# juliohm/GeoStatsSolvers.jl

Hardware: AMD Instinct MI355X
Metric: kriged domain points/sec (OK, 1000 3-D data, Matern-3/2, global neighbourhood) (higher is better)
Workload: dtype f64; 1 GPU; configs[1]: OK, 1000 3-D data -> 1000000 domain points per GPU, Matern-3/2 range 30, global neighbourhood; step = device fit + predict; points_per_gpu=1000000, ndata=1000, factor=replicated

## Files before the change

### geostatssolvers.jl_amd/csrc/krig.hip

```cpp
#include "gss_internal.h"
#include "cokrig.h"

#include <mutex>
#include "mfma_f64.h"

#include <cmath>
#include <cstdlib>
#include <cstring>
#include <type_traits>
#include <vector>

namespace gss {

constexpr int MAX_NC = 64;
constexpr int NSEG = 4;

struct DriftSpec {
  int variant;
  int nc;
  int dim;
  signed char e[MAX_NC][3];
  double center[3];
  double inv_scale[3];
};

template <int DIM>
__global__ __launch_bounds__(256) void drift_rows_kernel(DriftSpec ds, const double* __restrict__ x,
                                                         const double* __restrict__ drift_vals, int64_t npts,
                                                         int64_t ncols_pad, double* __restrict__ out, int64_t ld,
                                                         int nrows) {
  const int64_t p = (int64_t)blockIdx.x * 256 + threadIdx.x;
  if (p >= ncols_pad) return;
  const int64_t pc = p < npts ? p : npts - 1;
  double xs[DIM];
#pragma unroll
  for (int k = 0; k < DIM; ++k) xs[k] = (x[pc * DIM + k] - ds.center[k]) * ds.inv_scale[k];
  for (int c = 0; c < nrows; ++c) {
    double f = 0.0;
    if (c < ds.nc) {
      if (ds.variant == GSS_KRIG_ORDINARY) {
        f = 1.0;
      } else if (ds.variant == GSS_KRIG_UNIVERSAL) {
        f = 1.0;
#pragma unroll
        for (int k = 0; k < DIM; ++k)
          for (int q = 0; q < ds.e[c][k]; ++q) f *= xs[k];
      } else {
        f = drift_vals[pc * ds.nc + c];
      }
    }
    out[(int64_t)c * ld + p] = f;
  }
}

template <int KIND>
__device__ __forceinline__ double cov_d2_select(const VgDev& vg, double d2) {
  const double val = vg.cs * vg_shape(KIND, fmax(d2, 1e-300), vg.inv_range, vg.mscale, vg.pw);
  return d2 <= 0.0 ? vg.sill : val;
}

template <int DIM, int KIND>
__global__ __launch_bounds__(256) void krig_rhs2_kernel(VgDev vg, const double* __restrict__ xd, int n,
                                                        const double* __restrict__ x0, int64_t m_valid,
                                                        double* __restrict__ R, int64_t ldr, int seg_len, int nblk,
                                                        int64_t ncols) {
  for (int unit = blockIdx.x; unit < nblk * NSEG; unit += gridDim.x) {
    const int seg = unit % NSEG;
    const int64_t p = (int64_t)(unit / NSEG) * 512 + 2 * threadIdx.x;
    if (p >= ncols) continue;
    const int64_t pa = p < m_valid ? p : m_valid - 1, pb = p + 1 < m_valid ? p + 1 : m_valid - 1;
    double ca[DIM], cb[DIM];
#pragma unroll
    for (int k = 0; k < DIM; ++k) {
      ca[k] = x0[pa * DIM + k];
      cb[k] = x0[pb * DIM + k];
    }
    const int j0 = seg * seg_len;
    const int j1 = j0 + seg_len < n ? j0 + seg_len : n;
    double2* rp = reinterpret_cast<double2*>(R + (int64_t)j0 * ldr + p);
    const int64_t ld2 = ldr >> 1;
#pragma unroll 4
    for (int j = j0; j < j1; ++j) {
      double x[DIM];
#pragma unroll
      for (int k = 0; k < DIM; ++k) x[k] = xd[j * DIM + k];
      double2 v;
      if (KIND < 0) {
        v.x = cov_pair<DIM>(vg, x, ca);
        v.y = cov_pair<DIM>(vg, x, cb);
      } else {
        const double da = sqdist_nofma<DIM>(x, ca, vg.ir, true);
        const double db = sqdist_nofma<DIM>(x, cb, vg.ir, true);
        v.x = cov_d2_select < KIND < 0 ? 0 : KIND > (vg, da);
        v.y = cov_d2_select < KIND < 0 ? 0 : KIND > (vg, db);
      }
      *rp = v;
      rp += ld2;
    }
  }
}

template <int DIM>
static int32_t launch_krig_rhs(hipStream_t s, const VgDev& vg, const double* xd, int n, const double* x0,
                               int64_t m_valid, double* R, int64_t ldr, int seg_len, int nblk) {
  GSS_REQUIRE((ldr & 1) == 0, "launch_krig_rhs: odd leading dimension %lld (16-B stores need an even one)",
              (long long)ldr);
  const int64_t ncols = (int64_t)nblk * 256;
  const int nblk2 = (int)((ncols + 511) / 512);
  const dim3 g2((unsigned)(nblk2 * NSEG));
#define GSS_K1W_LAUNCH(KIND)                                                                                         \
  hipLaunchKernelGGL((krig_rhs2_kernel<DIM, KIND>), g2, dim3(256), 0, s, vg, xd, n, x0, m_valid, R, ldr, seg_len,    \
                     nblk2, ncols)
  switch (vg.nextra == 0 ? vg.kind : -1) {
    case GSS_VG_GAUSSIAN: GSS_K1W_LAUNCH(GSS_VG_GAUSSIAN); break;
    case GSS_VG_EXPONENTIAL: GSS_K1W_LAUNCH(GSS_VG_EXPONENTIAL); break;
    case GSS_VG_SPHERICAL: GSS_K1W_LAUNCH(GSS_VG_SPHERICAL); break;
    case VG_MATERN12: GSS_K1W_LAUNCH(VG_MATERN12); break;
    case VG_MATERN32: GSS_K1W_LAUNCH(VG_MATERN32); break;
    case VG_MATERN52: GSS_K1W_LAUNCH(VG_MATERN52); break;
    default: GSS_K1W_LAUNCH(-1); break;
  }
#undef GSS_K1W_LAUNCH
  return GSS_OK;
}


template <int DIM>
__global__ __launch_bounds__(256) void cokrig_system_kernel(VgDev vg, const double* __restrict__ xd,
                                                            const int* __restrict__ var,
                                                            const double* __restrict__ tab, int n,
                                                            double* __restrict__ M, int64_t ldw) {
  const int j = blockIdx.x * 256 + threadIdx.x;
  const int i0 = blockIdx.y * 64;
  const int i1 = i0 + 64 < n ? i0 + 64 : n;
  if (j >= n) return;
  double c[DIM];
#pragma unroll
  for (int k = 0; k < DIM; ++k) c[k] = xd[(int64_t)j * DIM + k];
  const int vj = var[j];
  for (int i = i0; i < i1; ++i) {
    double x[DIM];
#pragma unroll
    for (int k = 0; k < DIM; ++k) x[k] = xd[(int64_t)i * DIM + k];
    bool zero;
    const double rho = co_rho<DIM, -1>(vg, x, c, &zero);
    const int e = var[i] * CO_MAXZ + vj;
    M[(int64_t)i * ldw + j] = zero ? tab[CO_C0 + e] : tab[e] * rho;
  }
}

__global__ __launch_bounds__(256) void cokrig_indicator_kernel(const int* __restrict__ var, int n, int nc,
                                                               double* __restrict__ Fd) {
  const int i = blockIdx.x * 256 + threadIdx.x;
  if (i >= n) return;
  const int v = var[i];
  for (int c = 0; c < nc; ++c) Fd[(int64_t)c * n + i] = v == c ? 1.0 : 0.0;
}

__global__ __launch_bounds__(256) void cokrig_center_kernel(double* __restrict__ z, const int* __restrict__ var,
                                                            const double* __restrict__ tab, int n) {
  const int i = blockIdx.x * 256 + threadIdx.x;
  if (i < n) z[i] -= tab[CO_MEANS + var[i]];
}

template <int DIM, int KIND>
__global__ __launch_bounds__(256) void cokrig_rhs_kernel(VgDev vg, const double* __restrict__ xd,
                                                         const int* __restrict__ var, const double* __restrict__ tab,
// ... 185 lines not shown
  double macc[2] = {0.0, 0.0};

  int buf = 0;
  for (int I = Ibeg; I < Iend; ++I) {
    const int i0 = I * BM;
    const int tm_max = (N1 + 1 - i0 + 15) / 16 < 8 ? (N1 + 1 - i0 + 15) / 16 : 8;
    const int t0 = i0 / BK;

    const double* wp = W + (int64_t)kq * ldw + i0 + i2;
    const double* rp = R + (int64_t)kq * ldr + p0 + i2;
    if (I == Ibeg) {
      d2v ra[4], rb[4];
#pragma unroll
      for (int r = 0; r < 4; ++r) {
        ra[r] = *reinterpret_cast<const d2v*>(wp + (int64_t)(4 * r) * ldw);
        rb[r] = *reinterpret_cast<const d2v*>(rp + (int64_t)(4 * r) * ldr);
      }
#pragma unroll
      for (int r = 0; r < 4; ++r) {
        *reinterpret_cast<d2v*>(As + (kq + 4 * r) * LDS_LD + i2) = ra[r];
        *reinterpret_cast<d2v*>(Bs + (kq + 4 * r) * LDS_LD + i2) = rb[r];
      }
      __syncthreads();
    }

    auto row_block = [&](auto tmx) __attribute__((always_inline)) {
      constexpr int TM_MAX = decltype(tmx)::value;
      d4 accw[8][2];
#pragma unroll
      for (int tm = 0; tm < TM_MAX; ++tm) accw[tm][0] = accw[tm][1] = d4{0.0, 0.0, 0.0, 0.0};

      auto stage = [&](int t, auto tmn, auto is_last) __attribute__((always_inline)) {
        constexpr int TM_MIN = decltype(tmn)::value;
        constexpr bool last = decltype(is_last)::value;
        const int cur = buf;
        const bool more = !last || (I + 1 < Iend);
        d2v ra[4], rb[4];
        if (more) {
          const double* wq = last ? wp + BM : wp + (int64_t)(t + 1) * BK * ldw;
          const double* rq = last ? rp : rp + (int64_t)(t + 1) * BK * ldr;
#pragma unroll
          for (int r = 0; r < 4; ++r) {
            ra[r] = *reinterpret_cast<const d2v*>(wq + (int64_t)(4 * r) * ldw);
            rb[r] = *reinterpret_cast<const d2v*>(rq + (int64_t)(4 * r) * ldr);
          }
        }
        mma_stage_w14<TM_MIN, TM_MAX>(As + cur * TILE_LDS, Bs + cur * TILE_LDS, accw, wave, lane);
        if (more) {
          double* an = As + (cur ^ 1) * TILE_LDS;
          double* bn = Bs + (cur ^ 1) * TILE_LDS;
#pragma unroll
          for (int r = 0; r < 4; ++r) {
            *reinterpret_cast<d2v*>(an + (kq + 4 * r) * LDS_LD + i2) = ra[r];
            *reinterpret_cast<d2v*>(bn + (kq + 4 * r) * LDS_LD + i2) = rb[r];
          }
        }
        __syncthreads();
        buf ^= 1;
      };
      for (int t = 0; t < t0; ++t) stage(t, std::integral_constant<int, 0>{}, std::false_type{});
#define GSS_K3_DIAG_STAGE(S) \
  if constexpr (S < TM_MAX) stage(t0 + S, std::integral_constant<int, S>{}, std::bool_constant<S + 1 == TM_MAX>{})
      GSS_K3_DIAG_STAGE(0);
      GSS_K3_DIAG_STAGE(1);
      GSS_K3_DIAG_STAGE(2);
      GSS_K3_DIAG_STAGE(3);
      GSS_K3_DIAG_STAGE(4);
      GSS_K3_DIAG_STAGE(5);
      GSS_K3_DIAG_STAGE(6);
      GSS_K3_DIAG_STAGE(7);
#undef GSS_K3_DIAG_STAGE

#pragma unroll
      for (int tn = 0; tn < 2; ++tn) {
        double s = 0.0;
#pragma unroll
        for (int tm = 0; tm < TM_MAX; ++tm)
#pragma unroll
          for (int r = 0; r < 4; ++r) {
            const int row = i0 + tm * 16 + lk + 4 * r;
            const double v = accw[tm][tn][r];
            const double vv = v * v;
            s += (row < n) ? vv : (row < N1 ? -vv : 0.0);
            if (row == N1) macc[tn] += v;
          }
        qacc[tn] += s;
      }
    };
    switch (tm_max) {
      case 1: row_block(std::integral_constant<int, 1>{}); break;
      case 2: row_block(std::integral_constant<int, 2>{}); break;
      case 3: row_block(std::integral_constant<int, 3>{}); break;
      case 4: row_block(std::integral_constant<int, 4>{}); break;
      case 5: row_block(std::integral_constant<int, 5>{}); break;
      case 6: row_block(std::integral_constant<int, 6>{}); break;
      case 7: row_block(std::integral_constant<int, 7>{}); break;
      default: row_block(std::integral_constant<int, 8>{}); break;
    }
  }

#pragma unroll
  for (int tn = 0; tn < 2; ++tn) {
    qacc[tn] += __shfl_xor(qacc[tn], 16);
    qacc[tn] += __shfl_xor(qacc[tn], 32);
    macc[tn] += __shfl_xor(macc[tn], 16);
    macc[tn] += __shfl_xor(macc[tn], 32);
  }
  __syncthreads();
  double* red = smem;
  double* redm = smem + 2 * BN;
  if (lk == 0) {
    red[wave * 32 + lr] = qacc[0];
    red[wave * 32 + 16 + lr] = qacc[1];
    red[BN + wave * 32 + lr] = 0.0;
    red[BN + wave * 32 + 16 + lr] = 0.0;
    redm[wave * 32 + lr] = macc[0];
    redm[wave * 32 + 16 + lr] = macc[1];
    redm[BN + wave * 32 + lr] = 0.0;
    redm[BN + wave * 32 + 16 + lr] = 0.0;
  }
  __syncthreads();
  if (SPLIT) {
    if (tid < BN) {
      qpart[(int64_t)Ibeg * ldr + p0 + tid] = red[tid] + red[BN + tid];
      if (Ibeg == N1 / BM && p0 + tid < m_valid) mean_out[p0 + tid] = mean0 + (redm[tid] + redm[BN + tid]);
    }
    return;
  }
  if (tid < BN) {
    const int64_t p = p0 + tid;
    if (p < m_valid) {
      const double q = red[tid] + red[BN + tid];
      const double mu = mean0 + (redm[tid] + redm[BN + tid]);
      const double v = sill - q;
      mean_out[p] = mu;
      var_out[p] = v > 0.0 ? v : 0.0;
      if (status_out) status_out[p] = GSS_PT_OK;
    }
  }
}

__global__ __launch_bounds__(256) void krig_finish_kernel(const double* __restrict__ qpart, int nI, int64_t ldr,
                                                          double sill, int64_t m_valid, double* __restrict__ var_out,
                                                          uint8_t* __restrict__ status_out) {
  const int64_t p = (int64_t)blockIdx.x * 256 + threadIdx.x;
  if (p >= m_valid) return;
  double q = 0.0;
  for (int I = 0; I < nI; ++I) q += qpart[(int64_t)I * ldr + p];
  const double v = sill - q;
  var_out[p] = v > 0.0 ? v : 0.0;
  if (status_out) status_out[p] = GSS_PT_OK;
}

__global__ void flip_tail_kernel(double* u, int64_t from, int64_t to) {
  const int64_t i = from + (int64_t)blockIdx.x * 256 + threadIdx.x;
  if (i < to) u[i] = -u[i];
}

__global__ void flip_rows_kernel(double* u, int64_t ld, int64_t from, int64_t to, int64_t ncols) {
  const int64_t i = from + (int64_t)blockIdx.x * 256 + threadIdx.x;
  const int64_t c = blockIdx.y;
  if (i < to && c < ncols) u[i + c * ld] = -u[i + c * ld];
}

__global__ void add_scalar_kernel(double* x, int64_t n, double v) {
  const int64_t i = (int64_t)blockIdx.x * 256 + threadIdx.x;
  if (i < n) x[i] += v;
}

__global__ void sub_scalar_kernel(double* z, int64_t n, double mu) {
  const int64_t i = (int64_t)blockIdx.x * 256 + threadIdx.x;
  if (i < n) z[i] -= mu;
}

__global__ __launch_bounds__(256) void krig_loo_kernel(const double* __restrict__ Wp, int64_t ldw, int n, int N1,
                                                       const double* __restrict__ wd, const double* __restrict__ z,
                                                       double* __restrict__ pred, double* __restrict__ var,
                                                       uint8_t* __restrict__ status) {
  const int lane = threadIdx.x & 63;
  const int i = blockIdx.x * 4 + (threadIdx.x >> 6);
  if (i >= n) return;
  const double* col = Wp + (int64_t)i * ldw;
  double acc = 0.0;
  for (int k = i + lane; k < N1; k += 64) {
    const double w = col[k];
    acc = k < n ? fma(w, w, acc) : fma(-w, w, acc);
  }
#pragma unroll
  for (int off = 32; off >= 1; off >>= 1) acc += __shfl_xor(acc, off);
  if (lane != 0) return;
  const double NaN = __longlong_as_double(0x7ff8000000000000LL);
  const bool ok = acc > 0.0 && acc < __builtin_huge_val();
  const double v = 1.0 / acc;
  pred[i] = ok ? z[i] - wd[i] * v : NaN;
  var[i] = ok ? (v > 0.0 ? v : 0.0) : NaN;
  if (status) status[i] = ok ? GSS_PT_OK : GSS_PT_SINGULAR;
}

}

using namespace gss;

struct gss_krig {
  VgDev vg;
  int variant = GSS_KRIG_ORDINARY;
  double sk_mean = 0.0;
  int degree = 0;
  int ndrift = 0;
  int dim = 0;
  int64_t n = 0;
  int nc = 0;
  int64_t N1 = 0, N1pad = 0, ldw = 0;
  DriftSpec ds;
  DevBuf xdata, z, drift_data;
  Frame fr;
  DevBuf xraw;
  DevBuf factor;
  DevBuf fit_ws;
  hipEvent_t fit_done = nullptr;
  bool fit_pending = false;
  int* fit_info = nullptr;
  hipStream_t fit_stream = nullptr;
  bool fit_async = false;
  int* fit_info_host = nullptr;
  ~gss_krig() {
    if (fit_pending && fit_done) (void)hipEventSynchronize(fit_done);
    if (fit_done) (void)hipEventDestroy(fit_done);
    if (fit_info_host) (void)hipHostFree(fit_info_host);
  }
  bool factored = false;
  int block_nsub = 0;
  double block_cell[3] = {0.0, 0.0, 0.0};
  double block_cvv = 0.0;
  int nz = 0;
  DevBuf covar, cotab;
  double c00[CO_MAXZ] = {}, means[CO_MAXZ] = {};
  DevBuf co_xg, co_xg_raw, co_zres, co_row;
  int64_t co_off[CO_MAXZ + 1] = {};
  double* Wp() const { return factor.as<double>(); }
  double* wd() const { return factor.as<double>() + ldw * N1pad; }
};

namespace gss {
int32_t krig_local_dev(const VgDev& vg, int variant, int nc, int dim, const signed char* exps, double inv_scale,
                       double sk_mean, Searcher& sr, const double* xdata, const double* z, const double* drift_data,
                       const double* x0, const double* x0_raw, const double* drift_dom, int64_t m, int k,
                       int minneighbors, double* mean, double* var, uint8_t* status, int* idx_out, int* count_out,
                       hipStream_t s, HostPipe* pipe, int block_nsub, const double* block_cell, double block_cvv,
                       const KnnMask* mask = nullptr);
}


template <int DIM>
__global__ __launch_bounds__(256) void krig_rhs_block_kernel(VgDev vg, const double* __restrict__ xd, int n,
                                                             const double* __restrict__ x0, int64_t m_valid,
                                                             double* __restrict__ R, int64_t ldr, int nsub,
                                                             double c1, double c2, double c3) {
  const int64_t p = (int64_t)blockIdx.x * 256 + threadIdx.x;
  if (p >= ldr) return;
  const bool live = p < m_valid;
  double c[DIM];
#pragma unroll
  for (int a = 0; a < DIM; ++a) c[a] = live ? x0[p * DIM + a] : 0.0;
  const double cell[3] = {c1, c2, c3};
  const int ns = DIM == 1 ? nsub : (DIM == 2 ? nsub * nsub : nsub * nsub * nsub);
  const double inv = 1.0 / (double)ns;
  for (int j = 0; j < n; ++j) {
    double xj[DIM];
#pragma unroll
    for (int a = 0; a < DIM; ++a) xj[a] = xd[(int64_t)j * DIM + a];
    double acc = 0.0;
    for (int s = 0; s < ns; ++s) {
      int q = s;
      double sp[DIM];
#pragma unroll
      for (int a = DIM - 1; a >= 0; --a) {
        const int ia = q % nsub;
        q /= nsub;
        sp[a] = c[a] + (((double)ia + 0.5) / (double)nsub - 0.5) * cell[a];
      }
      acc += cov_pair<DIM>(vg, xj, sp);
    }
    R[(int64_t)j * ldr + p] = live ? acc * inv : 0.0;
  }
}

template <int DIM>
__global__ __launch_bounds__(256) void block_cvv_kernel(VgDev vg, int nsub, double c1, double c2, double c3,
                                                        double* __restrict__ out) {
  __shared__ double part[256];
  const double cell[3] = {c1, c2, c3};
  const int ns = DIM == 1 ? nsub : (DIM == 2 ? nsub * nsub : nsub * nsub * nsub);
  double acc = 0.0;
  for (int e = threadIdx.x; e < ns * ns; e += 256) {
    double a[DIM], b[DIM];
    int qa = e / ns, qb = e % ns;
#pragma unroll
    for (int d = DIM - 1; d >= 0; --d) {
      a[d] = (((double)(qa % nsub) + 0.5) / (double)nsub - 0.5) * cell[d];
      b[d] = (((double)(qb % nsub) + 0.5) / (double)nsub - 0.5) * cell[d];
      qa /= nsub;
      qb /= nsub;
    }
    acc += cov_pair<DIM>(vg, a, b);
  }
  part[threadIdx.x] = acc;
  __syncthreads();
  if (threadIdx.x == 0) {
    double t = 0.0;
    for (int i = 0; i < 256; ++i) t += part[i];
    *out = t / ((double)ns * (double)ns);
  }
}

static void uk_exponents(int dim, int degree, std::vector<signed char>& e) {
  e.clear();
  for (int total = 0; total <= degree; ++total) {
    int idx[3] = {0, 0, 0};
    const int lim = total + 1;
    const int cnt = (dim == 1) ? lim : (dim == 2 ? lim * lim : lim * lim * lim);
    for (int t = 0; t < cnt; ++t) {
      int r = t;
      for (int k = dim - 1; k >= 0; --k) {
        idx[k] = r % lim;
        r /= lim;
      }
      int sum = 0;
      for (int k = 0; k < dim; ++k) sum += idx[k];
      if (sum == total) {
        for (int k = 0; k < 3; ++k) e.push_back((signed char)(k < dim ? idx[k] : 0));
      }
    }
  }
}

static int64_t krig_chunk_points(int64_t N1pad, int64_t m) {
  size_t ws = (size_t)16 << 30;
  size_t freeb = 0, totalb = 0;
  if (hipMemGetInfo(&freeb, &totalb) == hipSuccess && freeb / 2 < ws) ws = freeb / 2;
  if (const char* e = std::getenv("GSS_KRIG_WS_MB")) {
    const long v = std::atol(e);
    if (v > 0) ws = (size_t)v << 20;
  }
  int64_t cap = (int64_t)(ws / (sizeof(double) * (size_t)N1pad));
  const int64_t round = 512 * 128;
  cap = cap >= round ? cap / round * round : cap / 256 * 256;
  if (cap < 256) cap = 256;
  return round_up(m, 256) < cap ? round_up(m, 256) : cap;
}

struct KrigWorkspace {
  DevBuf R, mean_part;
  int64_t doubles = 0, mc = 0, nI = 0;
};
static KrigWorkspace g_ws;

static int32_t krig_workspace(int64_t N1pad, int64_t mc, hipStream_t s, double** R, double** mean_part) {
  const int64_t nI = (N1pad + BM - 1) / BM + 1;
  if (g_ws.doubles < N1pad * mc || g_ws.mc < mc || g_ws.nI < nI) {
    GSS_HIP(hipStreamSynchronize(s));
    g_ws.R.release();
    g_ws.mean_part.release();
    GSS_TRY(g_ws.R.alloc(sizeof(double) * (size_t)(N1pad * mc)));
    GSS_TRY(g_ws.mean_part.alloc(sizeof(double) * (size_t)((NSEG + 1 + nI) * mc)));
    g_ws.doubles = N1pad * mc;
    g_ws.mc = mc;
    g_ws.nI = nI;
  }
  *R = g_ws.R.as<double>();
  *mean_part = g_ws.mean_part.as<double>();
  return GSS_OK;
}

static int32_t launch_drift_rows(const gss_krig* h, const double* x, const double* drift_vals, int64_t npts,
                                 int64_t ncols_pad, double* out, int64_t ld, int nrows, hipStream_t s) {
  dim3 grid((unsigned)((ncols_pad + 255) / 256));
  switch (h->dim) {
    case 1:
      hipLaunchKernelGGL((drift_rows_kernel<1>), grid, dim3(256), 0, s, h->ds, x, drift_vals, npts, ncols_pad, out,
                         ld, nrows);
      break;
    case 2:
      hipLaunchKernelGGL((drift_rows_kernel<2>), grid, dim3(256), 0, s, h->ds, x, drift_vals, npts, ncols_pad, out,
                         ld, nrows);
      break;
    default:
      hipLaunchKernelGGL((drift_rows_kernel<3>), grid, dim3(256), 0, s, h->ds, x, drift_vals, npts, ncols_pad, out,
                         ld, nrows);
      break;
  }
  GSS_HIP(hipGetLastError());
  return GSS_OK;
}

__global__ void small_gram_kernel(const double* __restrict__ Bm, int nc, int64_t n, double* __restrict__ S, int lds) {
  const int c = blockIdx.x, c2 = blockIdx.y;
  if (c2 > c) return;
  double acc = 0.0;
  for (int64_t i = threadIdx.x; i < n; i += 64) acc = fma(Bm[(int64_t)c * n + i], Bm[(int64_t)c2 * n + i], acc);
#pragma unroll
  for (int off = 32; off >= 1; off >>= 1) acc += __shfl_xor(acc, off);
  if (threadIdx.x == 0) {
    S[c + c2 * lds] = acc;
    S[c2 + c * lds] = acc;
  }
}

__global__ void constraint_rows_kernel(const double* __restrict__ WS, int64_t ldws, const double* __restrict__ T,
                                       int nc, int64_t n, double* __restrict__ Wp_rows, int64_t ldw) {
  const int64_t j = (int64_t)blockIdx.x * 256 + threadIdx.x;
  if (j >= n) return;
  for (int i = 0; i < nc; ++i) {
    double acc = 0.0;
    for (int c = 0; c <= i; ++c) acc = fma(WS[i + c * ldws], T[(int64_t)c * n + j], acc);
    Wp_rows[i + j * ldw] = -acc;
  }
}

__global__ __launch_bounds__(256) void wd_row_kernel(const double* __restrict__ wd, int64_t N1,
                                                     double* __restrict__ row, int64_t ldw) {
  const int64_t k = (int64_t)blockIdx.x * 256 + threadIdx.x;
  if (k < N1) row[k * ldw] = wd[k];
}

struct FitPlan {
  double *M, *T, *Dinv, *Fd, *Bm, *S, *SDinv, *gwork, *zz, *u;
  int *info, *info2;
  int64_t szM, szS;
};

static int32_t krig_fit_plan(gss_krig* h, FitPlan* fp) {
  const int64_t n = h->n, N1pad = h->N1pad, ldw = h->ldw;
  const int64_t szM = ldw * N1pad;
  int64_t szT = n * n > (int64_t)MAX_NC * n ? n * n : (int64_t)MAX_NC * n;
  if (potrf_inverse_work_doubles(n) > szT) szT = potrf_inverse_work_doubles(n);
  const int64_t szDinv = 64 * 64;
  const int64_t szFd = (int64_t)MAX_NC * n, szBm = (int64_t)MAX_NC * n;
  const int64_t szS = 2 * MAX_NC * MAX_NC + 64 * 64;
  int64_t szGemv = gemv_work_doubles(false, ldw, ldw);
  if (gemv_work_doubles(true, ldw, ldw) > szGemv) szGemv = gemv_work_doubles(true, ldw, ldw);
  const int64_t szVec = 2 * ldw;
  DevBuf& ws = h->fit_ws;
  GSS_TRY(ws.alloc(sizeof(double) * (size_t)(szM + szT + szDinv + szFd + szBm + szS + szGemv + szVec) + 64));
  fp->M = ws.as<double>();
  fp->T = fp->M + szM;
  fp->Dinv = fp->T + szT;
  fp->Fd = fp->Dinv + szDinv;
  fp->Bm = fp->Fd + szFd;
  fp->S = fp->Bm + szBm;
  fp->SDinv = fp->S + MAX_NC * MAX_NC;
  fp->gwork = fp->S + szS;
  fp->zz = fp->gwork + szGemv;
  fp->u = fp->zz + ldw;
  fp->info = reinterpret_cast<int*>(fp->u + ldw);
  fp->info2 = fp->info + 1;
  fp->szM = szM;
  fp->szS = szS;
  return GSS_OK;
}

static int32_t krig_fit_enqueue(gss_krig* h, const FitPlan& fp, hipStream_t s) {
  const int64_t n = h->n, N1 = h->N1, ldw = h->ldw;
  const int nc = h->nc;
  double *M = fp.M, *T = fp.T, *Fd = fp.Fd, *Bm = fp.Bm, *S = fp.S, *SDinv = fp.SDinv;
  double *gwork = fp.gwork, *zz = fp.zz, *u = fp.u;
  int *info = fp.info, *info2 = fp.info2;
  const int64_t szM = fp.szM, szS = fp.szS;
  GSS_TRY(dev_zero_bytes(M, sizeof(double) * (size_t)szM, s));
  GSS_TRY(dev_zero_bytes(h->factor.p, h->factor.bytes, s));
  GSS_TRY(dev_zero_bytes(info2, sizeof(int), s));
  if (h->nz > 0) {
    const dim3 grid((unsigned)((n + 255) / 256), (unsigned)((n + 63) / 64));
    switch (h->dim) {
      case 1: hipLaunchKernelGGL(cokrig_system_kernel<1>, grid, dim3(256), 0, s, h->vg, h->xdata.as<double>(), h->covar.as<int>(), h->cotab.as<double>(), (int)n, M, ldw); break;
      case 2: hipLaunchKernelGGL(cokrig_system_kernel<2>, grid, dim3(256), 0, s, h->vg, h->xdata.as<double>(), h->covar.as<int>(), h->cotab.as<double>(), (int)n, M, ldw); break;
      default: hipLaunchKernelGGL(cokrig_system_kernel<3>, grid, dim3(256), 0, s, h->vg, h->xdata.as<double>(), h->covar.as<int>(), h->cotab.as<double>(), (int)n, M, ldw); break;
    }
    GSS_HIP(hipGetLastError());
  } else {
    GSS_TRY(cov_pairwise_dev(h->vg, h->xdata.as<double>(), n, h->xdata.as<double>(), n, M, ldw, s));
  }
  double* Wp = h->Wp();
  GSS_TRY(potrf_inverse_f64(M, n, ldw, Wp, ldw, T, info, false, s, true));

  if (nc > 0) {
    GSS_TRY(dev_zero_bytes(S, sizeof(double) * (size_t)szS, s));
    if (h->nz > 0) {
      hipLaunchKernelGGL(cokrig_indicator_kernel, dim3((unsigned)((n + 255) / 256)), dim3(256), 0, s,
                         h->covar.as<int>(), (int)n, nc, Fd);
      GSS_HIP(hipGetLastError());
    } else {
      GSS_TRY(launch_drift_rows(h, h->xdata.as<double>(), h->drift_data.as<double>(), n, n, Fd, n, nc, s));
    }
    for (int c = 0; c < nc; ++c) GSS_TRY(gemv_f64(false, n, n, Wp, ldw, Fd + (int64_t)c * n, Bm + (int64_t)c * n, gwork, s));
    hipLaunchKernelGGL(small_gram_kernel, dim3(nc, nc), dim3(64), 0, s, Bm, nc, n, S, MAX_NC);
    GSS_HIP(hipGetLastError());
    GSS_TRY(potrf_inverse_f64(S, nc, MAX_NC, Wp + n + n * ldw, ldw, SDinv, info2, false, s));
    for (int c = 0; c < nc; ++c) GSS_TRY(gemv_f64(true, n, n, Wp, ldw, Bm + (int64_t)c * n, T + (int64_t)c * n, gwork, s));
    hipLaunchKernelGGL(constraint_rows_kernel, dim3((unsigned)((n + 255) / 256)), dim3(256), 0, s, Wp + n + n * ldw, ldw, T,
                       nc, n, Wp + n, ldw);
    GSS_HIP(hipGetLastError());
  }

  GSS_TRY(dev_zero_bytes(zz, sizeof(double) * (size_t)(2 * ldw), s));
  GSS_TRY(dev_copy_f64(zz, h->z.as<double>(), n, s));
  if (h->nz > 0) {
    if (h->variant == GSS_KRIG_SIMPLE)
      hipLaunchKernelGGL(cokrig_center_kernel, dim3((unsigned)((n + 255) / 256)), dim3(256), 0, s, zz,
                         h->covar.as<int>(), h->cotab.as<double>(), (int)n);
  } else if (h->variant == GSS_KRIG_SIMPLE && h->sk_mean != 0.0) {
    hipLaunchKernelGGL(sub_scalar_kernel, dim3((unsigned)((n + 255) / 256)), dim3(256), 0, s, zz, n, h->sk_mean);
  }
  GSS_TRY(gemv_f64(false, N1, N1, Wp, ldw, zz, u, gwork, s));
  if (nc > 0) hipLaunchKernelGGL(flip_tail_kernel, dim3(1), dim3(256), 0, s, u, n, N1);
  GSS_TRY(gemv_f64(true, N1, N1, Wp, ldw, u, h->wd(), gwork, s));
  hipLaunchKernelGGL(wd_row_kernel, dim3((unsigned)((N1 + 255) / 256)), dim3(256), 0, s, h->wd(), N1, Wp + N1, ldw);
  GSS_HIP(hipGetLastError());
  return GSS_OK;
}

static hipStream_t krig_fit_stream() { return helper_stream(HELPER_FIT); }

static int32_t krig_factor_alloc(gss_krig* h) {
  if (h->factor.p) return GSS_OK;
  return h->factor.alloc(sizeof(double) * (size_t)(h->ldw * h->N1pad + h->N1pad));
}

static int32_t krig_factorize(gss_krig* h, hipStream_t s, bool async = false) {
  GSS_TRY(krig_factor_alloc(h));
  hipStream_t fs = s;
  if (async) {
    fs = krig_fit_stream();
    if (!fs) {
      async = false;
      fs = s;
    }
  }
  if (async) {
    ScopedEvent e0;
    GSS_HIP(e0.create());
    GSS_HIP(hipEventRecord(e0, s));
    GSS_HIP(hipStreamWaitEvent(fs, e0, 0));
    if (!h->fit_info_host) GSS_HIP(hipHostMalloc(reinterpret_cast<void**>(&h->fit_info_host), 2 * sizeof(int), hipHostMallocDefault));
  }
  FitPlan fp;
  GSS_TRY(krig_fit_plan(h, &fp));
  GSS_TRY(krig_fit_enqueue(h, fp, fs));
  h->fit_info = fp.info;
  h->fit_stream = fs;
  h->fit_async = async;
  if (async) GSS_HIP(hipMemcpyAsync(h->fit_info_host, fp.info, 2 * sizeof(int), hipMemcpyDeviceToHost, fs));
  if (!h->fit_done) GSS_HIP(hipEventCreateWithFlags(&h->fit_done, hipEventDisableTiming));
  GSS_HIP(hipEventRecord(h->fit_done, fs));
  h->fit_pending = true;
  h->factored = true;
  return GSS_OK;
}

static int32_t krig_join_device(gss_krig* h, hipStream_t s) {
  if (h->fit_pending && h->fit_done && h->fit_stream != s) GSS_HIP(hipStreamWaitEvent(s, h->fit_done, 0));
  return GSS_OK;
}

static int32_t krig_fit_wait(gss_krig* h) {
  if (!h->fit_pending) return GSS_OK;
  h->fit_pending = false;
  GSS_HIP(hipEventSynchronize(h->fit_done));
  int hinfo[2] = {0, 0};
  if (h->fit_async) {
    hinfo[0] = h->fit_info_host[0];
    hinfo[1] = h->fit_info_host[1];
  } else {
    GSS_HIP(hipMemcpy(hinfo, h->fit_info, 2 * sizeof(int), hipMemcpyDeviceToHost));
  }
  h->fit_ws.release();
  h->fit_info = nullptr;
  if (hinfo[0] < 0) {
    h->factored = false;
    static thread_local bool retrying = false;
    if (!retrying) {
      potrf_panel_disable();
      retrying = true;
      int32_t rc = krig_factorize(h, h->fit_stream, false);
      if (rc == GSS_OK) rc = krig_fit_wait(h);
      retrying = false;
      return rc;
    }
    set_error("kriging fit: the factorisation kernel gave up waiting at a grid barrier");
    return GSS_ERR_HIP;
  }
  if (hinfo[0] != 0) {
    h->factored = false;
    set_error("kriging covariance matrix is not positive definite (pivot %d of %lld); add a nugget or remove "
              "duplicate samples", hinfo[0] - 1, (long long)h->n);
    return GSS_ERR_NOT_POSDEF;
  }
  if (hinfo[1] != 0) {
    h->factored = false;
    set_error("drift functions are linearly dependent on the sample locations (constraint %d)", hinfo[1] - 1);
    return GSS_ERR_NOT_POSDEF;
  }
  return GSS_OK;
}

static void launch_krig_quadform(const gss_krig* h, const double* Rws, int64_t ldr, double c00, double mean0,
                                 int64_t mv, int64_t cols, double* mean_out, double* var_out, uint8_t* stp,
                                 double* qpart, hipStream_t s) {
  const int nstrips = (int)(cols / BN);
  const int nI = (int)((h->N1 + BM) / BM);
#define GSS_K3_ARGS(S0, NS) h->Wp(), h->ldw, (int)h->N1pad, (int)h->n, (int)h->N1, Rws, ldr, c00, mean0, mv, \
                            mean_out, var_out, stp, qpart, (S0), (NS)
  const int nmain = (nstrips / 512) * 512;
  const int nrem = nstrips - nmain;
  if (nmain > 0)
    hipLaunchKernelGGL((krig_quadform_kernel<false>), dim3((unsigned)nmain), dim3(256), QUADFORM_LDS_BYTES, s,
                       GSS_K3_ARGS(0, nmain));
  if (nrem > 0) {
    const unsigned grid = (unsigned)(8 * ((nrem + 7) / 8) * nI);
    hipLaunchKernelGGL((krig_quadform_kernel<true>), dim3(grid), dim3(256), QUADFORM_LDS_BYTES, s,
                       GSS_K3_ARGS(nmain, nrem));
    const int64_t pbeg = (int64_t)nmain * BN;
    if (mv > pbeg)
      hipLaunchKernelGGL(krig_finish_kernel, dim3((unsigned)((mv - pbeg + 255) / 256)), dim3(256), 0, s, qpart + pbeg,
                         nI, ldr, c00, mv - pbeg, var_out + pbeg, stp ? stp + pbeg : nullptr);
  }
#undef GSS_K3_ARGS
}

static int32_t krig_quadform_attrs() {
  static uint64_t attr_set = 0;
  if (first_on_this_device(attr_set)) {
    GSS_HIP(hipFuncSetAttribute(reinterpret_cast<const void*>(krig_quadform_kernel<false>),
                                hipFuncAttributeMaxDynamicSharedMemorySize, (int)QUADFORM_LDS_BYTES));
    GSS_HIP(hipFuncSetAttribute(reinterpret_cast<const void*>(krig_quadform_kernel<true>),
                                hipFuncAttributeMaxDynamicSharedMemorySize, (int)QUADFORM_LDS_BYTES));
  }
  return GSS_OK;
}

static int32_t krig_refuse_cokrig(const gss_krig* h, const char* who) {
  GSS_REQUIRE(h->nz == 0, "%s: the handle is a cokriging system over %d variables; its estimates come from "
              "gss_cokrig_predict_global and gss_cokrig_predict_knn (cross-validation: gss_krig_cv_global, "
              "gss_krig_cv_global_folds, gss_cokrig_cv_knn)", who, h->nz);
  return GSS_OK;
}

extern "C" {

int32_t gss_krig_create(gss_krig_t** out, const gss_variogram_t* vg, int32_t variant, double sk_mean,
                        int32_t degree, int32_t ndrift, const double* xdata, const double* z,
                        const double* drift_data, int64_t n, int32_t flags, void* stream) {
  GSS_ENTRY();
  GSS_REQUIRE(out != nullptr, "gss_krig_create: out is NULL");
  *out = nullptr;
  GSS_REQUIRE(xdata != nullptr && z != nullptr, "gss_krig_create: NULL data");
  GSS_REQUIRE(n >= 1, "all samples are missing, aborting...");
  GSS_REQUIRE(n < (1 << 30), "too many samples");
  gss_krig* h = new (std::nothrow) gss_krig();
  if (!h) return GSS_ERR_ALLOC;
  struct Guard {
    gss_krig* h;
    ~Guard() { delete h; }
  } guard{h};
  gss_variogram_t plain;
  GSS_TRY(vg_frame_split(vg, &plain, &h->fr));
  GSS_TRY(make_vgdev(&plain, &h->vg));
  GSS_REQUIRE(variant != GSS_KRIG_SIMPLE || vg_is_stationary(vg),
              "simple kriging needs a stationary variogram (a power variogram has no sill)");
  GSS_TRY(frame_origin(&h->fr, xdata, GSS_MEM_HOST, nullptr));
// ... 926 lines not shown
```

Before: 52.35 million points/s.

## Fuse kriging fit tail into three custom kernels replacing gemv chain

Replaces the post-factorisation sequence (per-drift gemv calls, Gram kernel, small potrf, transposed gemvs, constraint rows, data-weight gemvs, flip and row-copy kernels) with three fused kernels. One batches the triangular products of all drift columns and centred data, one builds and factors the small constraint Gram block in shared memory, and one produces the constraint rows and data weights per column. The aim is to cut launch count and repeated passes over the n×n inverse factor during fit. It adds a custom in-shared-memory Cholesky with its own pivot threshold and restructures the workspace layout, which could shift numerics. For OK (nc=1) the fit is a small part of a step that predicts a million points, so the effect on the overall step is likely small.

Result: no change. 52.60 million points/s (median of 6 runs) (+0.5%).

```diff
diff --git a/geostatssolvers.jl_amd/csrc/krig.hip b/geostatssolvers.jl_amd/csrc/krig.hip
--- a/geostatssolvers.jl_amd/csrc/krig.hip
+++ b/geostatssolvers.jl_amd/csrc/krig.hip
@@ -3,6 +3,7 @@
 
 #include <mutex>
 #include "mfma_f64.h"
+#include "krig_fit_tail.h"
 
 #include <cmath>
 #include <cstdlib>
@@ -13,6 +14,7 @@
 namespace gss {
 
 constexpr int MAX_NC = 64;
+static_assert(TAIL_NC == MAX_NC, "krig_fit_tail.h sizes its constraint block for MAX_NC");
 constexpr int NSEG = 4;
 
 struct DriftSpec {
@@ -504,11 +506,6 @@
   if (status_out) status_out[p] = GSS_PT_OK;
 }
 
-__global__ void flip_tail_kernel(double* u, int64_t from, int64_t to) {
-  const int64_t i = from + (int64_t)blockIdx.x * 256 + threadIdx.x;
-  if (i < to) u[i] = -u[i];
-}
-
 __global__ void flip_rows_kernel(double* u, int64_t ld, int64_t from, int64_t to, int64_t ncols) {
   const int64_t i = from + (int64_t)blockIdx.x * 256 + threadIdx.x;
   const int64_t c = blockIdx.y;
@@ -518,11 +515,6 @@
 __global__ void add_scalar_kernel(double* x, int64_t n, double v) {
   const int64_t i = (int64_t)blockIdx.x * 256 + threadIdx.x;
   if (i < n) x[i] += v;
-}
-
-__global__ void sub_scalar_kernel(double* z, int64_t n, double mu) {
-  const int64_t i = (int64_t)blockIdx.x * 256 + threadIdx.x;
-  if (i < n) z[i] -= mu;
 }
 
 __global__ __launch_bounds__(256) void krig_loo_kernel(const double* __restrict__ Wp, int64_t ldw, int n, int N1,
@@ -745,82 +737,36 @@
   return GSS_OK;
 }
 
-__global__ void small_gram_kernel(const double* __restrict__ Bm, int nc, int64_t n, double* __restrict__ S, int lds) {
-  const int c = blockIdx.x, c2 = blockIdx.y;
-  if (c2 > c) return;
-  double acc = 0.0;
-  for (int64_t i = threadIdx.x; i < n; i += 64) acc = fma(Bm[(int64_t)c * n + i], Bm[(int64_t)c2 * n + i], acc);
-#pragma unroll
-  for (int off = 32; off >= 1; off >>= 1) acc += __shfl_xor(acc, off);
-  if (threadIdx.x == 0) {
-    S[c + c2 * lds] = acc;
-    S[c2 + c * lds] = acc;
-  }
-}
-
-__global__ void constraint_rows_kernel(const double* __restrict__ WS, int64_t ldws, const double* __restrict__ T,
-                                       int nc, int64_t n, double* __restrict__ Wp_rows, int64_t ldw) {
-  const int64_t j = (int64_t)blockIdx.x * 256 + threadIdx.x;
-  if (j >= n) return;
-  for (int i = 0; i < nc; ++i) {
-    double acc = 0.0;
-    for (int c = 0; c <= i; ++c) acc = fma(WS[i + c * ldws], T[(int64_t)c * n + j], acc);
-    Wp_rows[i + j * ldw] = -acc;
-  }
-}
-
-__global__ __launch_bounds__(256) void wd_row_kernel(const double* __restrict__ wd, int64_t N1,
-                                                     double* __restrict__ row, int64_t ldw) {
-  const int64_t k = (int64_t)blockIdx.x * 256 + threadIdx.x;
-  if (k < N1) row[k * ldw] = wd[k];
-}
-
 struct FitPlan {
-  double *M, *T, *Dinv, *Fd, *Bm, *S, *SDinv, *gwork, *zz, *u;
+  double *M, *T, *Fd, *X, *ub;
   int *info, *info2;
-  int64_t szM, szS;
+  int64_t zero_doubles;
 };
 
 static int32_t krig_fit_plan(gss_krig* h, FitPlan* fp) {
   const int64_t n = h->n, N1pad = h->N1pad, ldw = h->ldw;
-  const int64_t szM = ldw * N1pad;
-  int64_t szT = n * n > (int64_t)MAX_NC * n ? n * n : (int64_t)MAX_NC * n;
-  if (potrf_inverse_work_doubles(n) > szT) szT = potrf_inverse_work_doubles(n);
-  const int64_t szDinv = 64 * 64;
-  const int64_t szFd = (int64_t)MAX_NC * n, szBm = (int64_t)MAX_NC * n;
-  const int64_t szS = 2 * MAX_NC * MAX_NC + 64 * 64;
-  int64_t szGemv = gemv_work_doubles(false, ldw, ldw);
-  if (gemv_work_doubles(true, ldw, ldw) > szGemv) szGemv = gemv_work_doubles(true, ldw, ldw);
-  const int64_t szVec = 2 * ldw;
+  const int64_t szM = ldw * N1pad, szInfo = 8;
+  const int64_t szT = potrf_inverse_work_doubles(n) > n * n ? potrf_inverse_work_doubles(n) : n * n;
+  const int64_t szFd = (int64_t)MAX_NC * n, szX = (int64_t)(MAX_NC + 1) * n;
   DevBuf& ws = h->fit_ws;
-  GSS_TRY(ws.alloc(sizeof(double) * (size_t)(szM + szT + szDinv + szFd + szBm + szS + szGemv + szVec) + 64));
+  GSS_TRY(ws.alloc(sizeof(double) * (size_t)(szM + szInfo + szT + szFd + szX + MAX_NC)));
   fp->M = ws.as<double>();
-  fp->T = fp->M + szM;
-  fp->Dinv = fp->T + szT;
-  fp->Fd = fp->Dinv + szDinv;
-  fp->Bm = fp->Fd + szFd;
-  fp->S = fp->Bm + szBm;
-  fp->SDinv = fp->S + MAX_NC * MAX_NC;
-  fp->gwork = fp->S + szS;
-  fp->zz = fp->gwork + szGemv;
-  fp->u = fp->zz + ldw;
-  fp->info = reinterpret_cast<int*>(fp->u + ldw);
+  fp->info = reinterpret_cast<int*>(fp->M + szM);
   fp->info2 = fp->info + 1;
-  fp->szM = szM;
-  fp->szS = szS;
+  fp->T = fp->M + szM + szInfo;
+  fp->Fd = fp->T + szT;
+  fp->X = fp->Fd + szFd;
+  fp->ub = fp->X + szX;
+  fp->zero_doubles = szM + szInfo;
   return GSS_OK;
 }
 
 static int32_t krig_fit_enqueue(gss_krig* h, const FitPlan& fp, hipStream_t s) {
-  const int64_t n = h->n, N1 = h->N1, ldw = h->ldw;
+  const int64_t n = h->n, ldw = h->ldw;
   const int nc = h->nc;
-  double *M = fp.M, *T = fp.T, *Fd = fp.Fd, *Bm = fp.Bm, *S = fp.S, *SDinv = fp.SDinv;
-  double *gwork = fp.gwork, *zz = fp.zz, *u = fp.u;
-  int *info = fp.info, *info2 = fp.info2;
-  const int64_t szM = fp.szM, szS = fp.szS;
-  GSS_TRY(dev_zero_bytes(M, sizeof(double) * (size_t)szM, s));
+  double* M = fp.M;
+  GSS_TRY(dev_zero_bytes(M, sizeof(double) * (size_t)fp.zero_doubles, s));
   GSS_TRY(dev_zero_bytes(h->factor.p, h->factor.bytes, s));
-  GSS_TRY(dev_zero_bytes(info2, sizeof(int), s));
   if (h->nz > 0) {
     const dim3 grid((unsigned)((n + 255) / 256), (unsigned)((n + 63) / 64));
     switch (h->dim) {
@@ -833,40 +779,33 @@
     GSS_TRY(cov_pairwise_dev(h->vg, h->xdata.as<double>(), n, h->xdata.as<double>(), n, M, ldw, s));
   }
   double* Wp = h->Wp();
-  GSS_TRY(potrf_inverse_f64(M, n, ldw, Wp, ldw, T, info, false, s, true));
+  GSS_TRY(potrf_inverse_f64(M, n, ldw, Wp, ldw, fp.T, fp.info, false, s, true));
 
   if (nc > 0) {
-    GSS_TRY(dev_zero_bytes(S, sizeof(double) * (size_t)szS, s));
     if (h->nz > 0) {
       hipLaunchKernelGGL(cokrig_indicator_kernel, dim3((unsigned)((n + 255) / 256)), dim3(256), 0, s,
-                         h->covar.as<int>(), (int)n, nc, Fd);
+                         h->covar.as<int>(), (int)n, nc, fp.Fd);
       GSS_HIP(hipGetLastError());
     } else {
-      GSS_TRY(launch_drift_rows(h, h->xdata.as<double>(), h->drift_data.as<double>(), n, n, Fd, n, nc, s));
-    }
-    for (int c = 0; c < nc; ++c) GSS_TRY(gemv_f64(false, n, n, Wp, ldw, Fd + (int64_t)c * n, Bm + (int64_t)c * n, gwork, s));
-    hipLaunchKernelGGL(small_gram_kernel, dim3(nc, nc), dim3(64), 0, s, Bm, nc, n, S, MAX_NC);
-    GSS_HIP(hipGetLastError());
-    GSS_TRY(potrf_inverse_f64(S, nc, MAX_NC, Wp + n + n * ldw, ldw, SDinv, info2, false, s));
-    for (int c = 0; c < nc; ++c) GSS_TRY(gemv_f64(true, n, n, Wp, ldw, Bm + (int64_t)c * n, T + (int64_t)c * n, gwork, s));
-    hipLaunchKernelGGL(constraint_rows_kernel, dim3((unsigned)((n + 255) / 256)), dim3(256), 0, s, Wp + n + n * ldw, ldw, T,
-                       nc, n, Wp + n, ldw);
-    GSS_HIP(hipGetLastError());
-  }
-
-  GSS_TRY(dev_zero_bytes(zz, sizeof(double) * (size_t)(2 * ldw), s));
-  GSS_TRY(dev_copy_f64(zz, h->z.as<double>(), n, s));
+      GSS_TRY(launch_drift_rows(h, h->xdata.as<double>(), h->drift_data.as<double>(), n, n, fp.Fd, n, nc, s));
+    }
+  }
+  TailZ zs{h->z.as<double>(), nullptr, nullptr, 0.0};
   if (h->nz > 0) {
-    if (h->variant == GSS_KRIG_SIMPLE)
-      hipLaunchKernelGGL(cokrig_center_kernel, dim3((unsigned)((n + 255) / 256)), dim3(256), 0, s, zz,
-                         h->covar.as<int>(), h->cotab.as<double>(), (int)n);
-  } else if (h->variant == GSS_KRIG_SIMPLE && h->sk_mean != 0.0) {
-    hipLaunchKernelGGL(sub_scalar_kernel, dim3((unsigned)((n + 255) / 256)), dim3(256), 0, s, zz, n, h->sk_mean);
-  }
-  GSS_TRY(gemv_f64(false, N1, N1, Wp, ldw, zz, u, gwork, s));
-  if (nc > 0) hipLaunchKernelGGL(flip_tail_kernel, dim3(1), dim3(256), 0, s, u, n, N1);
-  GSS_TRY(gemv_f64(true, N1, N1, Wp, ldw, u, h->wd(), gwork, s));
-  hipLaunchKernelGGL(wd_row_kernel, dim3((unsigned)((N1 + 255) / 256)), dim3(256), 0, s, h->wd(), N1, Wp + N1, ldw);
+    if (h->variant == GSS_KRIG_SIMPLE) {
+      zs.var = h->covar.as<int>();
+      zs.tab = h->cotab.as<double>();
+    }
+  } else if (h->variant == GSS_KRIG_SIMPLE) {
+    zs.mean = h->sk_mean;
+  }
+  const unsigned nrb = (unsigned)((n + TAIL_ROWS - 1) / TAIL_ROWS), ncb = (unsigned)((n + TAIL_COLS - 1) / TAIL_COLS);
+  hipLaunchKernelGGL(krig_tail_rows_kernel, dim3(nrb, (unsigned)(nc / TAIL_CB + 1)), dim3(64 * TAIL_RWAVES), 0, s, Wp, ldw,
+                     (int)n, nc, nc > 0 ? fp.Fd : nullptr, zs, fp.X);
+  if (nc > 0)
+    hipLaunchKernelGGL(krig_tail_block_kernel, dim3(1), dim3(256), 0, s, fp.X, (int)n, nc, Wp, ldw, fp.ub, h->wd(),
+                       fp.info2);
+  hipLaunchKernelGGL(krig_tail_cols_kernel, dim3(ncb), dim3(256), 0, s, Wp, ldw, (int)n, nc, fp.X, fp.ub, h->wd());
   GSS_HIP(hipGetLastError());
   return GSS_OK;
 }
diff --git a/geostatssolvers.jl_amd/csrc/krig_fit_tail.h b/geostatssolvers.jl_amd/csrc/krig_fit_tail.h
--- /dev/null
+++ b/geostatssolvers.jl_amd/csrc/krig_fit_tail.h
@@ -0,0 +1,222 @@
+#pragma once
+
+#include "cokrig.h"
+
+namespace gss {
+
+constexpr int TAIL_NC = 64;
+constexpr int TAIL_LD = TAIL_NC + 1;
+constexpr int TAIL_CB = 8;
+constexpr int TAIL_ROWS = 64;
+constexpr int TAIL_RWAVES = 8;
+constexpr int TAIL_COLS = 8;
+constexpr int TAIL_XS = 3200;
+constexpr double TAIL_PIVOT_REL = 0x1p-40;
+constexpr int TAIL_ENT = ((TAIL_NC + 1) * (TAIL_NC + 2) / 2 + 255) / 256;
+
+struct TailZ {
+  const double* z;
+  const int* var;
+  const double* tab;
+  double mean;
+};
+
+__device__ __forceinline__ double tail_zc(const TailZ& zs, int j) {
+  return zs.z[j] - (zs.tab ? zs.tab[CO_MEANS + zs.var[j]] : zs.mean);
+}
+
+__device__ __forceinline__ double tail_wave_sum(double v) {
+#pragma unroll
+  for (int off = 32; off >= 1; off >>= 1) v += __shfl_xor(v, off);
+  return v;
+}
+
+__global__ __launch_bounds__(64 * TAIL_RWAVES) void krig_tail_rows_kernel(const double* __restrict__ Wp, int64_t ldw,
+                                                                          int n, int nc,
+                                                                          const double* __restrict__ Fd, TailZ zs,
+                                                                          double* __restrict__ X) {
+  __shared__ double part[TAIL_RWAVES][TAIL_CB][TAIL_ROWS];
+  const int lane = threadIdx.x & 63;
+  const int wave = __builtin_amdgcn_readfirstlane(threadIdx.x >> 6);
+  const int i0 = blockIdx.x * TAIL_ROWS, i = i0 + lane;
+  const int c0 = blockIdx.y * TAIL_CB;
+  const int jend = i0 + TAIL_ROWS < n ? i0 + TAIL_ROWS : n;
+  const double* wrow = Wp + (i < n ? i : n - 1);
+  double acc[TAIL_CB];
+#pragma unroll
+  for (int cc = 0; cc < TAIL_CB; ++cc) acc[cc] = 0.0;
+#pragma unroll 4
+  for (int j = wave; j < jend; j += TAIL_RWAVES) {
+    const double wv = wrow[(int64_t)j * ldw];
+    const double w = j <= i ? wv : 0.0;
+#pragma unroll
+    for (int cc = 0; cc < TAIL_CB; ++cc) {
+      const int c = c0 + cc;
+      if (c <= nc) acc[cc] = fma(w, c < nc ? Fd[(int64_t)c * n + j] : tail_zc(zs, j), acc[cc]);
+    }
+  }
+#pragma unroll
+  for (int cc = 0; cc < TAIL_CB; ++cc) part[wave][cc][lane] = acc[cc];
+  __syncthreads();
+  const int cc = threadIdx.x >> 6, c = c0 + cc;
+  if (c <= nc && i < n) {
+    double sum = 0.0;
+#pragma unroll
+    for (int w = 0; w < TAIL_RWAVES; ++w) sum += part[w][cc][lane];
+    X[(int64_t)c * n + i] = sum;
+  }
+}
+
+__global__ __launch_bounds__(256) void krig_tail_block_kernel(const double* __restrict__ X, int n, int nc,
+                                                              double* __restrict__ Wp, int64_t ldw,
+                                                              double* __restrict__ ub, double* __restrict__ wd,
+                                                              int* __restrict__ info) {
+  __shared__ double Ss[TAIL_LD * TAIL_LD];
+  __shared__ double Xs[TAIL_XS];
+  __shared__ double dg[TAIL_NC], us[TAIL_NC];
+  __shared__ unsigned short ents[TAIL_ENT * 256];
+  const int tid = threadIdx.x;
+  const int nr = nc + 1, nent = nr * (nr + 1) / 2;
+  const int ib = (TAIL_XS / nr - 1) / 32 * 32, ldx = ib + 1;
+  for (int e = tid; e < nent; e += 256) {
+    int c = 0;
+    while ((c + 1) * (c + 2) / 2 <= e) ++c;
+    const int c2 = e - c * (c + 1) / 2;
+    ents[e] = (unsigned short)((c << 8) | c2);
+    Ss[c * TAIL_LD + c2] = 0.0;
+  }
+  for (int p0 = 0; p0 < n; p0 += ib) {
+    const int len = p0 + ib < n ? ib : n - p0;
+    __syncthreads();
+    for (int q = tid; q < nr * len; q += 256) {
+      const int c = q / len, ii = q - c * len;
+      Xs[c * ldx + ii] = X[(int64_t)c * n + p0 + ii];
+    }
+    __syncthreads();
+#pragma unroll 1
+    for (int e = tid; e < nent; e += 256) {
+      const int c = ents[e] >> 8, c2 = ents[e] & 255;
+      const double* a = Xs + c * ldx;
+      const double* b = Xs + c2 * ldx;
+      double sum = Ss[c * TAIL_LD + c2];
+#pragma unroll 1
+      for (int s0 = 0; s0 < len; s0 += 32) {
+        const int s1 = s0 + 32 < len ? s0 + 32 : len;
+        double p = 0.0;
+#pragma unroll 8
+        for (int ii = s0; ii < s1; ++ii) p = fma(a[ii], b[ii], p);
+        sum += p;
+      }
+      Ss[c * TAIL_LD + c2] = sum;
+    }
+  }
+  __syncthreads();
+  int bad = 0;
+  for (int j = 0; j < nc; ++j) {
+    double v = 0.0;
+    if (tid >= j && tid < nc) {
+      const double s0 = Ss[tid * TAIL_LD + j];
+      v = s0;
+      for (int k = 0; k < j; ++k) v = fma(-Ss[tid * TAIL_LD + k], Ss[j * TAIL_LD + k], v);
+      dg[tid] = (tid == j && !(v > TAIL_PIVOT_REL * s0)) ? 0.0 : v;
+    }
+    __syncthreads();
+    double d = dg[j];
+    if (!(d > 0.0)) {
+      if (bad == 0) bad = j + 1;
+      d = 1.0;
+    }
+    const double l = sqrt(d);
+    if (tid >= j && tid < nc) Ss[tid * TAIL_LD + j] = tid == j ? l : v / l;
+    __syncthreads();
+  }
+  if (tid == 0 && bad != 0 && *info == 0) *info = bad;
+  if (tid < nc) {
+    const int c = tid;
+    const double x0 = 1.0 / Ss[c * TAIL_LD + c];
+    for (int i = c + 1; i < nc; ++i) {
+      double a = Ss[i * TAIL_LD + c] * x0;
+      for (int k = c + 1; k < i; ++k) a = fma(Ss[i * TAIL_LD + k], Ss[c * TAIL_LD + k], a);
+      Ss[c * TAIL_LD + i] = -a / Ss[i * TAIL_LD + i];
+    }
+  }
+  __syncthreads();
+  if (tid < nc) dg[tid] = 1.0 / Ss[tid * TAIL_LD + tid];
+  __syncthreads();
+  auto WS = [&](int i, int c) { return i == c ? dg[c] : Ss[c * TAIL_LD + i]; };
+  if (tid < nc) {
+    double a = 0.0;
+    for (int c = 0; c <= tid; ++c) a = fma(WS(tid, c), Ss[nc * TAIL_LD + c], a);
+    us[tid] = a;
+    ub[tid] = a;
+  }
+  __syncthreads();
+  if (tid < nc) {
+    double a = 0.0;
+    for (int k = tid; k < nc; ++k) a = fma(WS(k, tid), us[k], a);
+    wd[n + tid] = a;
+    Wp[(int64_t)(n + nc) + (int64_t)(n + tid) * ldw] = a;
+  }
+  for (int q = tid; q < nc * nc; q += 256) {
+    const int c = q / nc, i = q - c * nc;
+    if (i >= c) Wp[(int64_t)(n + i) + (int64_t)(n + c) * ldw] = WS(i, c);
+  }
+}
+
+__global__ __launch_bounds__(256) void krig_tail_cols_kernel(double* __restrict__ Wp, int64_t ldw, int n, int nc,
+                                                             const double* __restrict__ X,
+                                                             const double* __restrict__ ub,
+                                                             double* __restrict__ wd) {
+  __shared__ double WSs[TAIL_NC * TAIL_LD];
+  __shared__ double Ts[4][TAIL_LD + 1];
+  __shared__ double us[TAIL_NC];
+  const int lane = threadIdx.x & 63;
+  const int wave = __builtin_amdgcn_readfirstlane(threadIdx.x >> 6);
+  for (int q = threadIdx.x; q < nc * nc; q += 256) {
+    const int c = q / nc, i = q - c * nc;
+    WSs[i * TAIL_LD + c] = Wp[(int64_t)(n + i) + (int64_t)(n + c) * ldw];
+  }
+  if ((int)threadIdx.x < nc) us[threadIdx.x] = ub[threadIdx.x];
+  const int N1 = n + nc;
+  for (int q = 0; q < TAIL_COLS / 4; ++q) {
+    const int j = blockIdx.x * TAIL_COLS + 4 * q + wave;
+    const bool live = j < n;
+    const double* col = Wp + (int64_t)(live ? j : 0) * ldw;
+    for (int c0 = 0; c0 <= nc; c0 += TAIL_CB) {
+      double acc[TAIL_CB];
+#pragma unroll
+      for (int cc = 0; cc < TAIL_CB; ++cc) acc[cc] = 0.0;
+      if (live) {
+#pragma unroll 1
+        for (int k = j + lane; k < n; k += 64) {
+          const double w = col[k];
+#pragma unroll
+          for (int cc = 0; cc < TAIL_CB; ++cc)
+            if (c0 + cc <= nc) acc[cc] = fma(w, X[(int64_t)(c0 + cc) * n + k], acc[cc]);
+        }
+      }
+#pragma unroll
+      for (int cc = 0; cc < TAIL_CB; ++cc) {
+        const double t = tail_wave_sum(acc[cc]);
+        if (lane == 0 && c0 + cc <= nc) Ts[wave][c0 + cc] = t;
+      }
+    }
+    __syncthreads();
+    double r = 0.0;
+    if (live && lane < nc) {
+      double a = 0.0;
+      for (int c = 0; c <= lane; ++c) a = fma(WSs[lane * TAIL_LD + c], Ts[wave][c], a);
+      r = -a;
+      Wp[(int64_t)(n + lane) + (int64_t)j * ldw] = r;
+    }
+    const double tail = nc > 0 ? tail_wave_sum(lane < nc ? r * us[lane] : 0.0) : 0.0;
+    if (live && lane == 0) {
+      const double w = nc > 0 ? Ts[wave][nc] + tail : Ts[wave][nc];
+      wd[j] = w;
+      Wp[(int64_t)N1 + (int64_t)j * ldw] = w;
+    }
+    __syncthreads();
+  }
+}
+
+}
```
